# sxontheway/milliEye

Measured on AMD Instinct MI355X. Metric: frames/sec YOLOv3-416+fusion @batch32, 1/2/4/8 MI355X; mAP@0.5 vs ref, higher is better.
Workload: dtype f32; 1 GPU; yolov3.cfg 416x416 fp32 inference, batch=32 per GPU, full milliEye: Darknet.forward -> NMS -> Network.forward mode 0 (R-CNN head + radar fusion, 2 radar boxes/frame) -> output rows, synthetic frames U[0,1), deterministic trained-like weights; stage=full, batch_per_gpu=32, global_batch=32, img_size=416, parallelism=frames sharded over 1 GPU(s), one process per GPU, no data-path collective, rccl_ranks=0, full=False, output_rows_last_step=6449, rois_last_step=6449

## Files before the change

### millieye_amd/csrc/common.h

```cpp
#pragma once
#include <hip/hip_runtime.h>
#include <stdint.h>
#include <stdio.h>
#include <stdlib.h>
#include "millieye_hip.h"

namespace me {

void set_error(const char* fmt, ...);

inline int check_launch(const char* what) {
  hipError_t e = hipGetLastError();
  if (e != hipSuccess) {
    set_error("%s: %s", what, hipGetErrorString(e));
    return (int)e;
  }
  return 0;
}

inline bool aligned16(const void* p) { return (reinterpret_cast<uintptr_t>(p) & 15u) == 0; }

inline int64_t ceil_div(int64_t a, int64_t b) { return (a + b - 1) / b; }

inline int store_mode() {
  static const int mode = [] {
    const char* e = getenv("MILLIEYE_STORE_MODE");
    return e ? atoi(e) : 0;
  }();
  return mode;
}

typedef unsigned st_u32x4 __attribute__((ext_vector_type(4)));
__device__ __forceinline__ void store16(void* ptr, uint4 v, int mode) {
  if (mode == 0) {
    *reinterpret_cast<uint4*>(ptr) = v;
  } else {
    st_u32x4 d = {v.x, v.y, v.z, v.w};
    if (mode == 1)
      asm volatile("global_store_dwordx4 %0, %1, off nt" ::"v"(ptr), "v"(d) : "memory");
    else
      asm volatile("global_store_dwordx4 %0, %1, off sc1" ::"v"(ptr), "v"(d) : "memory");
  }
}
__device__ __forceinline__ void store4(float* ptr, float v, int mode) {
  if (mode == 0)
    *ptr = v;
  else
    __builtin_nontemporal_store(v, ptr);
}

}

#define ME_REQUIRE(cond, code, ...)   \
  do {                                \
    if (!(cond)) {                    \
      me::set_error(__VA_ARGS__);     \
      return (code);                  \
    }                                 \
  } while (0)

#define ME_HIP(call)                                                 \
  do {                                                               \
    hipError_t e__ = (call);                                         \
    if (e__ != hipSuccess) {                                         \
      me::set_error("%s failed: %s", #call, hipGetErrorString(e__)); \
      return (int)e__;                                               \
    }                                                                \
  } while (0)
```

### millieye_amd/csrc/conv.hip

```cpp
#include <stdlib.h>

#include "common.h"
#include "dma.h"

#include "conv32_common.h"

namespace me32 {
int launch_p8_tile(const ConvP& p, int tile, hipStream_t stream);
bool ws1x1_f32_eligible(const ConvP& p);
int launch_ws1x1_f32(const ConvP& p, hipStream_t stream);
bool ws3x3_f32_eligible(const ConvP& p);
int launch_ws3x3_f32(const ConvP& p, hipStream_t stream);
bool stem_mfma_eligible(const ConvP& p);
int launch_stem_mfma(const ConvP& p, hipStream_t stream);
}

namespace {

template <int BM, int BN, int BK, int WR, int WC, int ABL = 0, int PRIO = 0>
__global__ __launch_bounds__(256) void conv_igemm_f32(ConvP p) {
  static_assert(WR * WC == 4, "4 waves per workgroup");
  constexpr int TM = BM / WR, TN = BN / WC;
  constexpr int MT = TM / 32, NT = TN / 32;
  static_assert(MT >= 1 && NT >= 1, "wave tile must hold at least one 32x32 MFMA tile");
// ... 321 lines not shown
  const int a_row = (wr * TM + r32) * BK;
  const int b_row = (BM + wc * TN + r32) * BK;
  const int off0 = ((0 + hh) ^ sw) * 4, off1 = ((2 + hh) ^ sw) * 4;

  for (int s = 0; s < nstages; ++s) {
    if (s + 1 < nstages)
      asm volatile("s_waitcnt vmcnt(%0) lgkmcnt(0)" ::"n"(LPW) : "memory");
    else
      asm volatile("s_waitcnt vmcnt(0) lgkmcnt(0)" ::: "memory");
    __builtin_amdgcn_s_barrier();
    asm volatile("" ::: "memory");
    if (s + 2 < nstages) issue_stage((s + 2) % NST);
    if (DPRIO) __builtin_amdgcn_s_setprio(1);
    const float* Ab = smem + (s % NST) * STAGE_F + a_row;
    const float* Bb = smem + (s % NST) * STAGE_F + b_row;
    float4 af[2][MT], bf[2][NT];
#pragma unroll
    for (int half = 0; half < 2; ++half) {
      const int off = half ? off1 : off0;
#pragma unroll
      for (int i = 0; i < MT; ++i) af[half][i] = *reinterpret_cast<const float4*>(Ab + i * 32 * BK + off);
#pragma unroll
      for (int j = 0; j < NT; ++j) bf[half][j] = *reinterpret_cast<const float4*>(Bb + j * 32 * BK + off);
    }
    __builtin_amdgcn_sched_barrier(0);
#pragma unroll
    for (int half = 0; half < 2; ++half) {
#pragma unroll
      for (int kk = 0; kk < 4; ++kk)
#pragma unroll
        for (int i = 0; i < MT; ++i)
#pragma unroll
          for (int j = 0; j < NT; ++j) {
            const float4 av = af[half][i], bv = bf[half][j];
            const float a = kk == 0 ? av.x : kk == 1 ? av.y : kk == 2 ? av.z : av.w;
            const float b = kk == 0 ? bv.x : kk == 1 ? bv.y : kk == 2 ? bv.z : bv.w;
            acc[i][j] = __builtin_amdgcn_mfma_f32_32x32x2f32(a, b, acc[i][j], 0, 0, 0);
          }
    }
    if (DPRIO) __builtin_amdgcn_s_setprio(0);
  }

  if (p.splitk > 1) {
    float* slab = p.partial + (long long)sid * p.M * p.cout;
#pragma unroll
    for (int j = 0; j < NT; ++j) {
      const int co = n0 + wc * TN + j * 32 + r32;
#pragma unroll
      for (int i = 0; i < MT; ++i)
#pragma unroll
        for (int e = 0; e < 16; ++e) {
          const int m = m0 + wr * TM + i * 32 + (e & 3) + 8 * (e >> 2) + 4 * hh;
          if (co < p.cout && m < p.M) slab[(long long)m * p.cout + co] = acc[i][j][e];
        }
    }
    return;
  }
  const int hw = p.ho * p.wo;
#pragma unroll
  for (int j = 0; j < NT; ++j) {
    const int co = n0 + wc * TN + j * 32 + r32;
    const bool co_ok = co < p.cout;
    const float sc = co_ok ? p.scale[co] : 0.f;
    const float sh = co_ok ? p.shift[co] : 0.f;
#pragma unroll
    for (int i = 0; i < MT; ++i) {
#pragma unroll
      for (int e = 0; e < 16; ++e) {
        const int row = (e & 3) + 8 * (e >> 2) + 4 * hh;
        const int m = m0 + wr * TM + i * 32 + row;
        if (!co_ok || m >= p.M) continue;
        float v = apply_act(acc[i][j][e] * sc + sh, p.act);
        if (p.res) v += p.res[(long long)m * p.res_pitch + co];
        if (p.ups == 1) {
          p.y[(long long)m * p.y_pitch + co] = v;
        } else {
          const int nimg = m / hw;
          const int rem = m - nimg * hw;
          const int oy = rem / p.wo, ox = rem - oy * p.wo;
          const int W2 = p.wo * 2;
          const long long base = ((long long)nimg * (p.ho * 2) + 2 * oy) * W2 + 2 * ox;
          p.y[(base)*p.y_pitch + co] = v;
          p.y[(base + 1) * p.y_pitch + co] = v;
          p.y[(base + W2) * p.y_pitch + co] = v;
          p.y[(base + W2 + 1) * p.y_pitch + co] = v;
        }
      }
    }
  }
}

template <int CT>
__global__ __launch_bounds__(256) void conv_stem3_f32(ConvP p) {
  constexpr int K = 27;
  const int m = blockIdx.x * 256 + threadIdx.x;
  const int co0 = blockIdx.y * CT;
  if (m >= p.M) return;
  const int hw = p.ho * p.wo;
  const int nimg = m / hw;
  const int rem = m - nimg * hw;
  const int oy = rem / p.wo, ox = rem - oy * p.wo;
  float xin[K];
#pragma unroll
  for (int ky = 0; ky < 3; ++ky)
#pragma unroll
    for (int kx = 0; kx < 3; ++kx) {
      const int iy = oy * p.stride - p.pad + ky, ix = ox * p.stride - p.pad + kx;
      const bool ok = ((unsigned)iy < (unsigned)p.h) && ((unsigned)ix < (unsigned)p.w);
#pragma unroll
      for (int c = 0; c < 3; ++c) {
        float v = 0.f;
        if (ok)
          v = p.x_nchw ? p.x[(((long long)nimg * 3 + c) * p.h + iy) * p.w + ix]
                       : p.x[((long long)(nimg * p.h + iy) * p.w + ix) * p.x_pitch + c];
        xin[(ky * 3 + kx) * 3 + c] = v;
      }
    }
  const float* __restrict__ wg = p.wgt + (long long)co0 * K;
  float acc[CT];
#pragma unroll
  for (int j = 0; j < CT; ++j) {
    float a = 0.f;
#pragma unroll
    for (int k = 0; k < K; ++k) a = fmaf(xin[k], wg[j * K + k], a);
    acc[j] = apply_act(a * p.scale[co0 + j] + p.shift[co0 + j], p.act);
  }
  float* yrow = p.y + (long long)m * p.y_pitch + co0;
#pragma unroll
  for (int j = 0; j < CT; j += 4) *reinterpret_cast<float4*>(yrow + j) = make_float4(acc[j], acc[j + 1], acc[j + 2], acc[j + 3]);
}

using namespace me_dma;

__device__ __forceinline__ unsigned udiv_magic32(unsigned n, unsigned m, unsigned s) { return (__umulhi(n, m) + n) >> s; }

template <int N, class F, int I = 0>
__device__ __forceinline__ void static_for(F&& f) {
  if constexpr (I < N) {
    f(std::integral_constant<int, I>{});
    static_for<N, F, I + 1>(static_cast<F&&>(f));
  }
}

__device__ __forceinline__ void tile_coords(const ConvP& p, int t, int& tile_m, int& tile_n) {
  const int per_panel = p.tiles_m * p.gn;
  const int panel = t / per_panel;
  const int r = t - panel * per_panel;
  const int left = p.tiles_n - panel * p.gn;
  const int width = left < p.gn ? left : p.gn;
  tile_m = r / width;
  tile_n = panel * p.gn + (r - tile_m * width);
}

template <int BM, int BN, int WR, int WC, int MINW = 1, int BABL = 0, int HYB = 0, int KORD = 0, int DEEP = 0, int MASKED = 0>
__global__ __launch_bounds__(64 * WR * WC, MINW) void conv_igemm_buf_f32(ConvP p) {
  constexpr int NW = WR * WC;
  static_assert(NW == 4 || NW == 8, "4 or 8 waves per workgroup");
  constexpr int BK = 16, NST = DEEP ? (KORD ? 9 : 6) : 3;
  constexpr int DEPTH = NST - 1;
  constexpr int TM = BM / WR, TN = BN / WC;
  constexpr int MT = TM / 32, NT = TN / 32;
  constexpr int GA = BM / 16, G = (BM + BN) / 16;
  constexpr int LPW = (G + NW - 1) / NW;
  constexpr int LA = GA / NW;
  constexpr int STAGE_F = LPW * NW * 256;
  static_assert(GA % NW == 0, "A groups must split evenly over the waves");

  extern __shared__ __attribute__((aligned(16))) float smem[];
  const unsigned lds_base = (unsigned)(unsigned long long)(__attribute__((address_space(3))) float*)smem;

  const int tid = threadIdx.x;
  const int lane = tid & 63;
  const int wave = __builtin_amdgcn_readfirstlane(tid >> 6);
  const int wr = wave / WC, wc = wave % WC;
  const int r32 = lane & 31, hh = lane >> 5;

  int tile_m, tile_n;
  int sid = blockIdx.y;
  int piece = -1;
  {
    int nwg = p.tiles_m * p.tiles_n;
    int bid = blockIdx.x;
    int first = 0, per = 1;
    if constexpr (HYB) {
      if (bid < p.bulk) {
        nwg = p.bulk;
      } else {
        bid -= p.bulk;
        first = p.bulk;
        per = p.splitk;
        nwg = (nwg - p.bulk) * p.splitk;
      }
    }
    const int q = nwg >> 3, r = nwg & 7;
    const int xcd = bid & 7, idx = bid >> 3;
    int wg = (xcd < r ? xcd * (q + 1) : r * (q + 1) + (xcd - r) * q) + idx;
    if constexpr (HYB) {
      if (first || p.bulk == 0) {
        piece = wg;
        sid = wg % per;
        wg = first + wg / per;
      } else {
        sid = 0;
      }
    }
    tile_coords(p, wg, tile_m, tile_n);
    tile_m = __builtin_amdgcn_readfirstlane(tile_m);
    tile_n = __builtin_amdgcn_readfirstlane(tile_n);
  }
  const int m0 = tile_m * BM, n0 = tile_n * BN;
  const int hw = p.ho * p.wo;

  const int img0 = (int)udiv_magic32((unsigned)m0, p.hw_m, p.hw_s);
  const long long img_elems = (long long)p.h * p.w * p.x_pitch;
  const long long bias_elems = ((long long)p.pad * p.w + p.pad) * p.x_pitch;
  const u32x4 rsrc_a = make_rsrc(p.x + (long long)img0 * img_elems - bias_elems);
  const bool b_tiled = p.wgt_tiled != nullptr;
  const u32x4 rsrc_b = make_rsrc(b_tiled ? p.wgt_tiled + (long long)n0 * 16 : p.wgt + (long long)n0 * p.ktot);
  const unsigned b_row = b_tiled ? 64u : (unsigned)p.ktot * 4u;
  const unsigned b_step = b_tiled ? (unsigned)p.cout * 64u : BK * 4u;

  const int lrow = lane >> 2;
  unsigned v_base[LPW];
  constexpr bool KS3 = KORD == 1;
  unsigned v_pad[LA];
  unsigned v_cur[LPW];
#pragma unroll
  for (int j = 0; j < LPW; ++j) {
    const int g = wave + NW * j;
    const int row = g * 16 + lrow;
    const int q = (lane & 3) ^ ((row >> 2) & 3);
    v_base[j] = kOobOffset;
    if (j < LA) {
      unsigned padmask = 0xFFFFFFFFu;
      const int m = m0 + row;
      if (m < p.M) {
        const int nimg = (int)udiv_magic32((unsigned)m, p.hw_m, p.hw_s);
        const int rem = m - nimg * hw;
        const int oy = (int)udiv_magic32((unsigned)rem, p.wo_m, p.wo_s), ox = rem - oy * p.wo;
        const int iy0 = oy * p.stride - p.pad, ix0 = ox * p.stride - p.pad;
        unsigned ok = 0;
        auto in_w = [&](int kx) { return (unsigned)(ix0 + kx) < (unsigned)p.w ? 1u : 0u; };
        auto in_h = [&](int ky) { return (unsigned)(iy0 + ky) < (unsigned)p.h; };
        if (KS3 || p.ks == 3) {
          const unsigned cols = in_w(0) | in_w(1) << 1 | in_w(2) << 2;
          ok = (in_h(0) ? cols : 0u) | (in_h(1) ? cols << 3 : 0u) | (in_h(2) ? cols << 6 : 0u);
        } else if (p.ks == 1) {
          ok = in_h(0) ? in_w(0) : 0u;
        } else {
          unsigned cols = 0;
          for (int kx = 0; kx < p.ks; ++kx) cols |= in_w(kx) << kx;
          for (int ky = 0; ky < p.ks; ++ky) ok |= (in_h(ky) ? cols : 0u) << (ky * p.ks);
        }
        padmask = ~ok;
        const long long e = (long long)(nimg - img0) * img_elems + ((long long)iy0 * p.w + ix0) * p.x_pitch + bias_elems;
        v_base[j] = (unsigned)(e * 4) + 16u * q;
      }
      v_pad[j] = padmask;
    } else if (g < G) {
      const int co_local = row - BM;
      if (n0 + co_local < p.cout) v_base[j] = (unsigned)co_local * b_row + 16u * q;
    }
    v_cur[j] = BABL == 1 ? kOobOffset : v_base[j];
  }

  int s_begin = sid * p.sps;
  int s_end = (s_begin + p.sps < p.stages) ? s_begin + p.sps : p.stages;
  if constexpr (HYB) {
    if (piece < 0) {
      s_begin = 0;
      s_end = p.stages;
    }
  }
  f32x16 acc[MT][NT];
#pragma unroll
  for (int i = 0; i < MT; ++i)
#pragma unroll
    for (int j = 0; j < NT; ++j)
#pragma unroll
      for (int e = 0; e < 16; ++e) acc[i][j][e] = 0.f;

  constexpr unsigned STAGE_B = STAGE_F * 4u;
  const unsigned wave_lds = __builtin_amdgcn_readfirstlane(lds_base + (unsigned)wave * 1024u);
  const unsigned pitch4 = (unsigned)p.x_pitch * 4u;
  const int sw = (r32 >> 2) & 3;
  const int off0 = ((0 + hh) ^ sw) * 4, off1 = ((2 + hh) ^ sw) * 4;
  const float* a_frag = smem + (wr * TM + r32) * BK;
  const float* b_frag = smem + (BM + wc * TN + r32) * BK;

  auto compute_stage = [&](const float* Ab, const float* Bb) {
    if (MT * NT >= 4) __builtin_amdgcn_s_setprio(1);
    float4 af[2][MT], bf[2][NT];
#pragma unroll
    for (int half = 0; half < 2; ++half) {
      const int off = half ? off1 : off0;
#pragma unroll
      for (int i = 0; i < MT; ++i) af[half][i] = *reinterpret_cast<const float4*>(Ab + i * 32 * BK + off);
#pragma unroll
      for (int j = 0; j < NT; ++j) bf[half][j] = *reinterpret_cast<const float4*>(Bb + j * 32 * BK + off);
    }
    __builtin_amdgcn_sched_barrier(0);
#pragma unroll
    for (int half = 0; half < 2; ++half) {
#pragma unroll
      for (int kk = 0; kk < 4; ++kk)
#pragma unroll
        for (int i = 0; i < MT; ++i)
#pragma unroll
// ... 31 lines not shown
      b_off = (unsigned)tap * (unsigned)p.cs * b_step;
    };
    enter_tap();
    a_off += (unsigned)cc * (BK * 4u);
    b_off += (unsigned)cc * b_step;
    auto issue_stage = [&](unsigned lds_dst) {
      dma_stage<LPW, LA, NW * 1024>(v_cur, rsrc_a, rsrc_b, __builtin_amdgcn_readfirstlane(a_off),
                                    __builtin_amdgcn_readfirstlane(b_off), lds_dst);
      a_off += BK * 4u;
      b_off += b_step;
      if (++cc == p.cs) {
        cc = 0;
        do {
          ++tap;
          if (++kx == p.ks) {
            kx = 0;
            ++ky;
          }
        } while (MASKED && tap < p.ks * p.ks && !((tmask >> tap) & 1u));
        enter_tap();
      }
    };
    const int nstages = s_end - s_begin;
    for (int i = 0; i < DEPTH && i < nstages; ++i) issue_stage(wave_lds + (unsigned)i * STAGE_B);
    auto wait_landed = [&](int younger) {
      bool done = false;
      static_for<DEPTH>([&](auto r_c) {
        constexpr int R = decltype(r_c)::value;
        if (!done && younger <= R) {
          asm volatile("s_waitcnt vmcnt(%0) lgkmcnt(0)" ::"n"(LPW * R) : "memory");
          done = true;
        }
      });
      if (!done) asm volatile("s_waitcnt vmcnt(%0) lgkmcnt(0)" ::"n"(LPW * (DEPTH - 1)) : "memory");
    };
    auto step = [&](auto slot_c) {
      constexpr int SLOT = decltype(slot_c)::value;
      asm volatile("s_waitcnt vmcnt(%0) lgkmcnt(0)" ::"n"(LPW * (DEPTH - 1)) : "memory");
      __builtin_amdgcn_s_barrier();
      asm volatile("" ::: "memory");
      issue_stage(wave_lds + ((SLOT + DEPTH) % NST) * STAGE_B);
      compute_stage(a_frag + SLOT * STAGE_F, b_frag + SLOT * STAGE_F);
    };
    int s = 0;
    for (; s + NST <= nstages - DEPTH; s += NST) static_for<NST>(step);
    int slot = 0;
    for (; s < nstages; ++s) {
      wait_landed(nstages - 1 - s);
      __builtin_amdgcn_s_barrier();
      asm volatile("" ::: "memory");
      if (s + DEPTH < nstages) issue_stage(wave_lds + (slot == 0 ? NST - 1 : slot - 1) * STAGE_B);
      compute_stage(a_frag + slot * STAGE_F, b_frag + slot * STAGE_F);
      slot = slot == NST - 1 ? 0 : slot + 1;
    }
  } else {
    unsigned v_tap[9][LPW];
    unsigned a_tap[9], b_tap[9];
#pragma unroll
    for (int t = 0; t < 9; ++t) {
#pragma unroll
      for (int j = 0; j < LPW; ++j)
        v_tap[t][j] = j < LA ? ((BABL == 1 || ((v_pad[j < LA ? j : 0] >> t) & 1u)) ? kOobOffset : v_base[j]) : v_cur[j];
      a_tap[t] = (unsigned)((t / 3) * p.w + (t % 3)) * pitch4;
      b_tap[t] = (unsigned)t * (unsigned)p.cs * b_step;
    }
    const int c_begin = s_begin / 9, c_end = s_end / 9;
    unsigned ca = (unsigned)c_begin * (BK * 4u), cb = (unsigned)c_begin * b_step;
    auto issue = [&](auto tap_c, unsigned ca_, unsigned cb_, unsigned lds_dst) {
      constexpr int T = decltype(tap_c)::value;
      dma_stage<LPW, LA, NW * 1024>(v_tap[T], rsrc_a, rsrc_b, __builtin_amdgcn_readfirstlane(a_tap[T] + ca_),
                                    __builtin_amdgcn_readfirstlane(b_tap[T] + cb_), lds_dst);
    };
    auto step = [&](auto tap_c, auto last_c) {
      constexpr int T = decltype(tap_c)::value;
      constexpr bool LAST = decltype(last_c)::value;
      constexpr int SLOT = T % NST;
      constexpr int YOUNGER = (LAST && 8 - T < DEPTH - 1) ? 8 - T : DEPTH - 1;
      asm volatile("s_waitcnt vmcnt(%0) lgkmcnt(0)" ::"n"(LPW * YOUNGER) : "memory");
      __builtin_amdgcn_s_barrier();
      asm volatile("" ::: "memory");
      constexpr unsigned DST = ((SLOT + DEPTH) % NST) * STAGE_B;
      if constexpr (T + DEPTH < 9)
        issue(std::integral_constant<int, (T + DEPTH) % 9>{}, ca, cb, wave_lds + DST);
      else if constexpr (!LAST)
        issue(std::integral_constant<int, (T + DEPTH) % 9>{}, ca + BK * 4u, cb + b_step, wave_lds + DST);
      compute_stage(a_frag + SLOT * STAGE_F, b_frag + SLOT * STAGE_F);
    };
    auto chunk = [&](auto last_c) { static_for<9>([&](auto tap_c) { step(tap_c, last_c); }); };
    static_for<DEPTH>([&](auto tap_c) { issue(tap_c, ca, cb, wave_lds + decltype(tap_c)::value * STAGE_B); });
    for (int c = c_begin; c + 1 < c_end; ++c) {
      chunk(std::false_type{});
      ca += BK * 4u;
      cb += b_step;
    }
    chunk(std::true_type{});
  }

  const bool split = HYB ? piece >= 0 : p.splitk > 1;
  if (split) {
    const long long slab_stride = HYB ? (long long)(BM * BN) : (long long)p.M * p.cout;
    float* slab0 = HYB ? p.partial + (long long)(piece - sid) * (BM * BN) : p.partial;
    auto slab_index = [&](int i, int j, int e, long long& idx) {
      const int lm = wr * TM + i * 32 + (e & 3) + 8 * (e >> 2) + 4 * hh, lc = wc * TN + j * 32 + r32;
      if (HYB) {
        idx = (long long)lm * BN + lc;
        return true;
      }
      idx = (long long)(m0 + lm) * p.cout + (n0 + lc);
      return m0 + lm < p.M && n0 + lc < p.cout;
    };
    float* mine = slab0 + (long long)sid * slab_stride;
#pragma unroll
    for (int j = 0; j < NT; ++j)
#pragma unroll
      for (int i = 0; i < MT; ++i)
#pragma unroll
        for (int e = 0; e < 16; ++e) {
          long long idx;
          if (!slab_index(i, j, e, idx)) continue;
          if (p.counters)
            __hip_atomic_store(mine + idx, acc[i][j][e], __ATOMIC_RELAXED, __HIP_MEMORY_SCOPE_AGENT);
          else
            mine[idx] = acc[i][j][e];
        }
    if (p.counters == nullptr) return;
    asm volatile("s_waitcnt vmcnt(0)" ::: "memory");
    __syncthreads();
    int* last_flag = reinterpret_cast<int*>(smem);
    if (tid == 0) {
      int* cnt = p.counters + (HYB ? piece / p.splitk : tile_m * p.tiles_n + tile_n);
      const int ticket = __hip_atomic_fetch_add(cnt, 1, __ATOMIC_RELAXED, __HIP_MEMORY_SCOPE_AGENT);
      const int last = ticket == p.splitk - 1;
      if (last) __hip_atomic_store(cnt, 0, __ATOMIC_RELAXED, __HIP_MEMORY_SCOPE_AGENT);
      *last_flag = last;
    }
    __syncthreads();
    if (*last_flag == 0) return;
#pragma unroll
    for (int j = 0; j < NT; ++j)
#pragma unroll
      for (int i = 0; i < MT; ++i)
#pragma unroll
        for (int e = 0; e < 16; ++e) {
          long long idx;
          if (!slab_index(i, j, e, idx)) continue;
          float a = __hip_atomic_load(slab0 + idx, __ATOMIC_RELAXED, __HIP_MEMORY_SCOPE_AGENT);
          for (int k = 1; k < p.splitk; ++k)
            a += __hip_atomic_load(slab0 + (long long)k * slab_stride + idx, __ATOMIC_RELAXED, __HIP_MEMORY_SCOPE_AGENT);
          acc[i][j][e] = a;
        }
  }
  if (m0 + BM <= p.M && n0 + BN <= p.cout && p.ups == 1 && p.act != ME_ACT_SIGMOID) {
    const float slope = p.act == ME_ACT_LEAKY ? 0.1f : 1.0f;
    const long long ystep = p.y_pitch, rstep = p.res_pitch;
#pragma unroll
    for (int j = 0; j < NT; ++j) {
      const int co = n0 + wc * TN + j * 32 + r32;
      const float sc = p.scale[co], sh = p.shift[co];
#pragma unroll
      for (int i = 0; i < MT; ++i) {
        const long long row0 = m0 + wr * TM + i * 32 + 4 * hh;
        float* yp = p.y + row0 * ystep + co;
        if (p.res) {
          const float* rp = p.res + row0 * rstep + co;
#pragma unroll
          for (int e = 0; e < 16; ++e) {
            const float t = acc[i][j][e] * sc + sh;
            me::store4(yp, fmaxf(t, t * slope) + *rp, p.store_mode);
            yp += (e & 3) == 3 ? 5 * ystep : ystep;
            rp += (e & 3) == 3 ? 5 * rstep : rstep;
          }
        } else {
#pragma unroll
          for (int e = 0; e < 16; ++e) {
            const float t = acc[i][j][e] * sc + sh;
            me::store4(yp, fmaxf(t, t * slope), p.store_mode);
            yp += (e & 3) == 3 ? 5 * ystep : ystep;
          }
        }
      }
    }
    return;
  }
#pragma unroll
  for (int j = 0; j < NT; ++j) {
    const int co = n0 + wc * TN + j * 32 + r32;
    const bool co_ok = co < p.cout;
    const float sc = co_ok ? p.scale[co] : 0.f;
    const float sh = co_ok ? p.shift[co] : 0.f;
#pragma unroll
    for (int i = 0; i < MT; ++i) {
#pragma unroll
      for (int e = 0; e < 16; ++e) {
        const int row = (e & 3) + 8 * (e >> 2) + 4 * hh;
        const int m = m0 + wr * TM + i * 32 + row;
        if (!co_ok || m >= p.M) continue;
        float v = apply_act(acc[i][j][e] * sc + sh, p.act);
        if (p.res) v += p.res[(long long)m * p.res_pitch + co];
        if (p.ups == 1) {
          p.y[(long long)m * p.y_pitch + co] = v;
        } else {
          const int nimg = m / hw;
          const int rem = m - nimg * hw;
          const int oy = rem / p.wo, ox = rem - oy * p.wo;
          const int W2 = p.wo * 2;
          const long long base = ((long long)nimg * (p.ho * 2) + 2 * oy) * W2 + 2 * ox;
          p.y[(base)*p.y_pitch + co] = v;
          p.y[(base + 1) * p.y_pitch + co] = v;
          p.y[(base + W2) * p.y_pitch + co] = v;
          p.y[(base + W2 + 1) * p.y_pitch + co] = v;
        }
      }
    }
  }
}

__global__ __launch_bounds__(256) void conv_splitk_reduce_f32(ConvP p) {
  const long long total = (long long)p.M * p.cout;
  const int hw = p.ho * p.wo;
  for (long long idx = (long long)blockIdx.x * 256 + threadIdx.x; idx < total; idx += (long long)gridDim.x * 256) {
    const int co = (int)(idx % p.cout);
    const int m = (int)(idx / p.cout);
    float a = p.partial[idx];
    for (int k = 1; k < p.splitk; ++k) a += p.partial[(long long)k * total + idx];
    float v = apply_act(a * p.scale[co] + p.shift[co], p.act);
    if (p.res) v += p.res[(long long)m * p.res_pitch + co];
    if (p.ups == 1) {
      p.y[(long long)m * p.y_pitch + co] = v;
    } else {
      const int nimg = m / hw;
      const int rem = m - nimg * hw;
      const int oy = rem / p.wo, ox = rem - oy * p.wo;
      const int W2 = p.wo * 2;
      const long long base = ((long long)nimg * (p.ho * 2) + 2 * oy) * W2 + 2 * ox;
      p.y[(base)*p.y_pitch + co] = v;
      p.y[(base + 1) * p.y_pitch + co] = v;
      p.y[(base + W2) * p.y_pitch + co] = v;
      p.y[(base + W2 + 1) * p.y_pitch + co] = v;
    }
  }
}

__global__ __launch_bounds__(256) void conv_tail_reduce_f32(ConvP p, int bm, int bn) {
  const int tile_elems = bm * bn;
  const long long total = (long long)(p.tiles_m * p.tiles_n - p.bulk) * tile_elems;
  const int hw = p.ho * p.wo;
  for (long long idx = (long long)blockIdx.x * 256 + threadIdx.x; idx < total; idx += (long long)gridDim.x * 256) {
    const int t = (int)(idx / tile_elems);
    const int rem_e = (int)(idx - (long long)t * tile_elems);
    const int lm = rem_e / bn, lc = rem_e - lm * bn;
    int tile_m, tile_n;
    tile_coords(p, p.bulk + t, tile_m, tile_n);
    const int m = tile_m * bm + lm;
    const int co = tile_n * bn + lc;
    if (m >= p.M || co >= p.cout) continue;
    const float* src = p.partial + (long long)t * p.splitk * tile_elems + rem_e;
    float a = src[0];
    for (int k = 1; k < p.splitk; ++k) a += src[(long long)k * tile_elems];
    float v = apply_act(a * p.scale[co] + p.shift[co], p.act);
    if (p.res) v += p.res[(long long)m * p.res_pitch + co];
    if (p.ups == 1) {
      p.y[(long long)m * p.y_pitch + co] = v;
    } else {
      const int nimg = m / hw;
      const int rem = m - nimg * hw;
      const int oy = rem / p.wo, ox = rem - oy * p.wo;
      const int W2 = p.wo * 2;
      const long long base = ((long long)nimg * (p.ho * 2) + 2 * oy) * W2 + 2 * ox;
      p.y[(base)*p.y_pitch + co] = v;
      p.y[(base + 1) * p.y_pitch + co] = v;
      p.y[(base + W2) * p.y_pitch + co] = v;
      p.y[(base + W2 + 1) * p.y_pitch + co] = v;
    }
  }
}

constexpr int SC_MAXCOUT = 128;

template <int CIN>
__global__ __launch_bounds__(256) void conv_smallcin_f32(ConvP p) {
  constexpr int K = 9 * CIN;
  __shared__ __attribute__((aligned(16))) float w_lds[K * SC_MAXCOUT];
  const int cout_pad = (p.cout + 7) & ~7;
  for (int idx = threadIdx.x; idx < K * cout_pad; idx += 256) {
    const int k = idx / cout_pad, co = idx - k * cout_pad;
    const int t = k / CIN, c = k - t * CIN;
    w_lds[idx] = (co < p.cout && c < p.cin) ? p.wgt[(long long)co * (9 * p.cin) + t * p.cin + c] : 0.f;
  }
  __syncthreads();

  const int tpp = cout_pad >> 3;
  const long long gid = (long long)blockIdx.x * 256 + threadIdx.x;
  const int m = (int)(gid / tpp);
  const int co0 = (int)(gid - (long long)m * tpp) * 8;
  if (m >= p.M) return;
  const int hw = p.ho * p.wo;
  const int nimg = m / hw;
  const int rem = m - nimg * hw;
  const int oy = rem / p.wo, ox = rem - oy * p.wo;

  float xin[K];
#pragma unroll
  for (int ky = 0; ky < 3; ++ky)
#pragma unroll
    for (int kx = 0; kx < 3; ++kx) {
      const int iy = oy * p.stride - p.pad + ky, ix = ox * p.stride - p.pad + kx;
// ... 205 lines not shown
  return a_max < (1ll << 31) && b_max < (1ll << 31) && b_tiled_max < (1ll << 31) && (long long)p.x_pitch * 4 < (1ll << 31);
}

void magic_u32(unsigned d, unsigned* m, unsigned* s) {
  unsigned sh = 0;
  while ((1ull << sh) < d) ++sh;
  *s = sh;
  *m = (unsigned)(((1ull << 32) * ((1ull << sh) - d)) / d + 1);
}

template <int BN>
void choose_order(ConvP& p) {
  static const long long kPanelBytes = [] {
    const char* e = getenv("MILLIEYE_PANEL_KB");
    return (e && atoi(e) > 0 ? (long long)atoi(e) : 1300ll) * 1024;
  }();
  static const int kChunkMajor = [] {
    const char* e = getenv("MILLIEYE_KORD");
    return e ? atoi(e) : 2;
  }();
  const long long col_bytes = (long long)BN * p.ktot * 4;
  p.gn = p.tiles_n;
  p.kord = (p.ks == 3 && p.cs >= 4 && kChunkMajor == 2) ? 1 : 0;
  if (col_bytes * p.tiles_n > kPanelBytes) {
    const long long fit = kPanelBytes / col_bytes;
    p.gn = fit < 1 ? 1 : fit > p.tiles_n ? p.tiles_n : (int)fit;
    if (p.ks == 3 && kChunkMajor >= 1) p.kord = 1;
  }
}

template <int BM, int BN, int WR, int WC, int MINW, int BABL, int HYB, int KORD, int DEEP = 0, int MASKED = 0>
int launch_buf_kernel(const ConvP& p, dim3 grid, hipStream_t stream) {
  constexpr int NW = WR * WC;
  constexpr int LPW = ((BM + BN) / 16 + NW - 1) / NW;
  constexpr int NST = DEEP ? (KORD ? 9 : 6) : 3;
  const size_t lds = (size_t)NST * LPW * NW * 256 * sizeof(float);
  auto kern = conv_igemm_buf_f32<BM, BN, WR, WC, MINW, BABL, HYB, KORD, DEEP, MASKED>;
  if (lds > 64 * 1024) {
    static bool attr_set = false;
    if (!attr_set) {
      ME_HIP(hipFuncSetAttribute(reinterpret_cast<const void*>(kern), hipFuncAttributeMaxDynamicSharedMemorySize,
                                 (int)lds));
      attr_set = true;
    }
  }
  hipLaunchKernelGGL(kern, grid, dim3(64 * NW), lds, stream, p);
  return me::check_launch(HYB ? "conv_igemm_buf_f32<tail split>" : "conv_igemm_buf_f32");
}

template <int BM, int BN, int WR, int WC, int MINW = 1, int BABL = 0, int DEEP = 0>
int launch_buf(ConvP& p, hipStream_t stream) {
  if (p.ks * p.ks > 32) {
    if constexpr (WR * WC == 4)
      return launch_igemm<BM, BN, 16, WR, WC>(p, stream);
    else
      return launch_igemm<128, 128, 16, 2, 2>(p, stream);
  }
  if (p.mask_cols)
    ME_REQUIRE(buf_addressable<BM>(p) && p.mask_cols % BN == 0 && BABL == 0 && DEEP == 0, ME_E_BADARG,
               "me_conv2d_f32: tap masks need cin %% 16 == 0, offsets below 2^31 and a tile width (%d) that divides tap_mask_cols", BN);
  if (!buf_addressable<BM>(p)) return launch_dma<BM, BN, WR, WC, 1, MINW>(p, stream);
  constexpr int BK = 16;
  p.cs = (p.cin + BK - 1) / BK;
  p.stages = p.ks * p.ks * p.cs;
  p.tiles_m = (p.M + BM - 1) / BM;
  p.tiles_n = (p.cout + BN - 1) / BN;
  choose_order<BN>(p);
  if (BABL || p.mask_cols) p.kord = 0;
  plan_split(p);
  const long long blocks = (long long)p.tiles_m * p.tiles_n;
  ME_REQUIRE(blocks < (1ll << 31), ME_E_TOOBIG, "me_conv2d_f32: grid too large");
  const dim3 grid((unsigned)blocks, (unsigned)p.splitk);
  if (blocks > p.counters_len || p.splitk == 1) p.counters = nullptr;
  int rc;
  if constexpr (BABL == 0) {
    if (p.mask_cols) {
      if constexpr (DEEP == 0) rc = launch_buf_kernel<BM, BN, WR, WC, MINW, 0, 0, 0, 0, 1>(p, grid, stream);
      else rc = ME_E_BADARG;
    } else
      rc = p.kord ? launch_buf_kernel<BM, BN, WR, WC, MINW, 0, 0, 1, DEEP>(p, grid, stream)
                  : launch_buf_kernel<BM, BN, WR, WC, MINW, 0, 0, 0, DEEP>(p, grid, stream);
  } else {
    rc = launch_buf_kernel<BM, BN, WR, WC, MINW, BABL, 0, 0>(p, grid, stream);
  }
  if (rc || p.splitk == 1 || p.counters) return rc;
  long long rb = ((long long)p.M * p.cout + 255) / 256;
  if (rb > 256 * 16) rb = 256 * 16;
  hipLaunchKernelGGL(conv_splitk_reduce_f32, dim3((unsigned)rb), dim3(256), 0, stream, p);
  return me::check_launch("conv_splitk_reduce_f32");
}

template <int BM, int BN, int WR, int WC, int MINW = 1, int DEEP = 0>
int launch_buf_tail(ConvP& p, hipStream_t stream, long long ws_bytes) {
  ME_REQUIRE(p.ks * p.ks <= 32 && buf_addressable<BM>(p), ME_E_BADARG,
             "me_conv2d_f32: the tail-split tiles need cin %% 16 == 0 and offsets below 2^31");
  constexpr int BK = 16;
  p.cs = (p.cin + BK - 1) / BK;
  p.stages = p.ks * p.ks * p.cs;
  p.tiles_m = (p.M + BM - 1) / BM;
  p.tiles_n = (p.cout + BN - 1) / BN;
  choose_order<BN>(p);
  const long long tiles = (long long)p.tiles_m * p.tiles_n;
  ME_REQUIRE(tiles < (1ll << 24), ME_E_TOOBIG, "me_conv2d_f32: grid too large");
  plan_split(p);
  p.bulk = (int)(tiles / 256 * 256);
  const long long tail = tiles - p.bulk;
  if (tail == 0 || p.splitk <= 1) {
    p.splitk = 1;
    p.bulk = 0;
    return launch_buf<BM, BN, WR, WC, MINW, 0, DEEP>(p, stream);
  }
  const long long need = tail * p.splitk * BM * BN * (long long)sizeof(float);
  ME_REQUIRE(p.partial && ws_bytes >= need, ME_E_BADARG, "me_conv2d_f32: tail split %d needs a workspace of %lld bytes",
             p.splitk, need);
  const dim3 grid((unsigned)(p.bulk + tail * p.splitk));
  if (tail > p.counters_len) p.counters = nullptr;
  int rc = p.kord ? launch_buf_kernel<BM, BN, WR, WC, MINW, 0, 1, 1, DEEP>(p, grid, stream)
                  : launch_buf_kernel<BM, BN, WR, WC, MINW, 0, 1, 0, DEEP>(p, grid, stream);
  if (rc || p.counters) return rc;
  long long rb = (tail * BM * BN + 255) / 256;
  if (rb > 256 * 16) rb = 256 * 16;
  hipLaunchKernelGGL(conv_tail_reduce_f32, dim3((unsigned)rb), dim3(256), 0, stream, p, BM, BN);
  return me::check_launch("conv_tail_reduce_f32");
}

int fill_params(const me_conv_desc* d, ConvP& p) {
  p.store_mode = me::store_mode();
  ME_REQUIRE(d != nullptr, ME_E_NULLPTR, "me_conv2d_f32: null descriptor");
  ME_REQUIRE(d->n > 0 && d->h > 0 && d->w > 0 && d->cin > 0 && d->cout > 0, ME_E_BADARG,
             "me_conv2d_f32: non-positive dimension");
  ME_REQUIRE(d->ksize >= 1 && d->stride >= 1 && d->pad >= 0, ME_E_BADARG, "me_conv2d_f32: bad ksize/stride/pad");
  const int ho = (d->h + 2 * d->pad - d->ksize) / d->stride + 1;
  const int wo = (d->w + 2 * d->pad - d->ksize) / d->stride + 1;
  ME_REQUIRE(ho == d->ho && wo == d->wo, ME_E_BADARG, "me_conv2d_f32: ho/wo (%d,%d) != derived (%d,%d)", d->ho,
             d->wo, ho, wo);
  ME_REQUIRE((long long)d->n * d->ho * d->wo < (1ll << 31), ME_E_TOOBIG, "me_conv2d_f32: too many output pixels");
  p.x = d->x; p.wgt = d->wgt; p.wgt_tiled = d->wgt_tiled; p.scale = d->scale; p.shift = d->shift; p.res = d->res; p.y = d->y;
  p.x_pitch = d->x_pitch; p.res_pitch = d->res_pitch; p.y_pitch = d->y_pitch;
  p.n = d->n; p.h = d->h; p.w = d->w; p.cin = d->cin; p.cout = d->cout; p.ks = d->ksize;
  p.stride = d->stride; p.pad = d->pad; p.ho = d->ho; p.wo = d->wo; p.act = d->act; p.ups = d->upsample;
  p.x_nchw = d->x_nchw;
  p.M = d->n * d->ho * d->wo;
  p.ktot = d->ksize * d->ksize * d->cin;
  magic_u32((unsigned)(d->ho * d->wo), &p.hw_m, &p.hw_s);
  magic_u32((unsigned)d->wo, &p.wo_m, &p.wo_s);
  p.cs = p.stages = p.tiles_m = p.tiles_n = p.bulk = p.gn = p.kord = 0;
  p.partial = nullptr;
  p.splitk = 1;
  p.sps = 0;
  p.counters = d->tile_counters_len > 0 ? d->tile_counters : nullptr;
  p.counters_len = p.counters ? d->tile_counters_len : 0;
  p.mask_cols = d->tap_mask_cols > 0 ? d->tap_mask_cols : 0;
  for (int i = 0; i < 4; ++i) p.tapmask[i] = d->tap_mask[i];
  return 0;
}

}

extern "C" {

int64_t me_conv2d_flops(const me_conv_desc* d) {
  if (!d) return 0;
  return 2ll * d->n * d->ho * d->wo * (int64_t)d->cout * d->ksize * d->ksize * d->cin;
}

int64_t me_conv2d_workspace_bytes(const me_conv_desc* d) {
  ConvP p;
  if (!d || fill_params(d, p) != 0 || d->cin <= 4) return 0;
  if ((d->tile >= 41 && d->tile <= 45) || d->tile == 47) {
    static const int shape[7][2] = {{128, 128}, {128, 64}, {64, 64}, {128, 32}, {256, 128}, {0, 0}, {64, 64}};
    const int bm = shape[d->tile - 41][0], bn = shape[d->tile - 41][1];
    const long long tiles = (long long)((p.M + bm - 1) / bm) * ((p.cout + bn - 1) / bn);
    const int split = d->split_k > 0 ? d->split_k : 4;
    return (int64_t)(tiles % 256) * split * bm * bn * (int64_t)sizeof(float);
  }
  const ConvPlan plan = plan_conv(p, d->tile, d->split_k > 0 ? d->split_k : kMaxSplit);
  const int split = d->split_k > 0 ? d->split_k : plan.splitk;
  return split > 1 ? (int64_t)split * p.M * p.cout * (int64_t)sizeof(float) : 0;
}

int me_conv2d_f32(const me_conv_desc* d, void* stream_) {
  hipStream_t stream = reinterpret_cast<hipStream_t>(stream_);
  ConvP p;
  int rc = fill_params(d, p);
  if (rc) return rc;
  ME_REQUIRE(d->x && d->wgt && d->scale && d->shift && d->y, ME_E_NULLPTR, "me_conv2d_f32: null tensor pointer");
  ME_REQUIRE(d->upsample == 1 || d->upsample == 2, ME_E_BADARG, "me_conv2d_f32: upsample must be 1 or 2");
  ME_REQUIRE(d->act >= 0 && d->act <= 2, ME_E_BADARG, "me_conv2d_f32: unknown activation %d", d->act);
  ME_REQUIRE(d->y_pitch >= d->cout, ME_E_BADARG, "me_conv2d_f32: y_pitch < cout");

  if (d->cin <= 4) {
    ME_REQUIRE(d->ksize == 3, ME_E_BADARG, "me_conv2d_f32: cin <= 4 needs ksize 3 (direct stem kernel)");
    ME_REQUIRE(d->cout <= SC_MAXCOUT, ME_E_TOOBIG, "me_conv2d_f32: small-cin kernel supports cout <= %d", SC_MAXCOUT);
    ME_REQUIRE(d->res == nullptr && d->upsample == 1, ME_E_BADARG,
               "me_conv2d_f32: small-cin kernel has no residual/upsample epilogue");
    ME_REQUIRE(d->x_nchw || d->x_pitch >= d->cin, ME_E_BADARG, "me_conv2d_f32: x_pitch < cin");
    ME_REQUIRE(me::aligned16(d->y), ME_E_ALIGN, "me_conv2d_f32: y not 16-byte aligned");
    if (d->tile == 0 && me32::stem_mfma_eligible(p)) return me32::launch_stem_mfma(p, stream);
    if (d->cin == 3 && (d->y_pitch & 3) == 0 && d->tile != 91) {
      const unsigned mb = (unsigned)((p.M + 255) / 256);
      if (d->cout % 32 == 0) {
        hipLaunchKernelGGL(conv_stem3_f32<32>, dim3(mb, d->cout / 32), dim3(256), 0, stream, p);
        return me::check_launch("conv_stem3_f32");
      }
      if (d->cout % 16 == 0) {
        hipLaunchKernelGGL(conv_stem3_f32<16>, dim3(mb, d->cout / 16), dim3(256), 0, stream, p);
        return me::check_launch("conv_stem3_f32");
      }
    }
    const long long threads = (long long)p.M * (((p.cout + 7) & ~7) >> 3);
    const unsigned blocks = (unsigned)((threads + 255) / 256);
    if (d->cin == 3)
      hipLaunchKernelGGL(conv_smallcin_f32<3>, dim3(blocks), dim3(256), 0, stream, p);
    else
      hipLaunchKernelGGL(conv_smallcin_f32<4>, dim3(blocks), dim3(256), 0, stream, p);
    return me::check_launch("conv_smallcin_f32");
  }

  ME_REQUIRE(!d->x_nchw, ME_E_BADARG, "me_conv2d_f32: NCHW input only supported for cin <= 4");
  ME_REQUIRE(d->cin % 4 == 0, ME_E_BADARG, "me_conv2d_f32: cin %% 4 != 0 (cin=%d)", d->cin);
  ME_REQUIRE(d->x_pitch >= d->cin && d->x_pitch % 4 == 0, ME_E_ALIGN, "me_conv2d_f32: x_pitch must be >= cin, %% 4");
  ME_REQUIRE(me::aligned16(d->x) && me::aligned16(d->wgt), ME_E_ALIGN, "me_conv2d_f32: x / wgt not 16-byte aligned");
  ME_REQUIRE(!d->res || d->res_pitch >= d->cout, ME_E_BADARG, "me_conv2d_f32: res_pitch < cout");
  ME_REQUIRE(d->split_k >= 0 && d->split_k <= 64, ME_E_BADARG, "me_conv2d_f32: split_k out of range");

  if (p.mask_cols) {
    const int taps = d->ksize * d->ksize, classes = d->cout / p.mask_cols;
    ME_REQUIRE(taps <= 16 && d->cout % p.mask_cols == 0 && classes >= 1 && classes <= 4 && d->upsample == 1 && d->split_k <= 1 &&
                   d->tile >= 0 && d->tile <= 5 && d->cin % 16 == 0, ME_E_BADARG,
               "me_conv2d_f32: tap masks need ksize^2 <= 16, 1 - 4 column classes, upsample 1, split_k <= 1, tile 0 - 5, cin %% 16 == 0");
    for (int i = 0; i < classes; ++i)
      ME_REQUIRE((d->tap_mask[i] & ((1u << taps) - 1u)) != 0, ME_E_BADARG, "me_conv2d_f32: tap_mask[%d] selects no tap", i);
    p.splitk = 1;
    p.partial = nullptr;
    int tile = d->tile;
    if (tile == 0) tile = p.mask_cols % 128 == 0 ? 1 : p.mask_cols % 64 == 0 ? 2 : 4;
    switch (tile) {
      case 1: return launch_buf<128, 128, 2, 2>(p, stream);
      case 2: return launch_buf<128, 64, 2, 2>(p, stream);
      case 3: return launch_buf<64, 64, 2, 2>(p, stream);
      case 4: return launch_buf<128, 32, 4, 1>(p, stream);
      default: return launch_buf<256, 128, 4, 2, 4>(p, stream);
    }
  }

  if ((d->tile >= 41 && d->tile <= 45) || d->tile == 47) {
    p.splitk = d->split_k > 0 ? d->split_k : 4;
    p.partial = reinterpret_cast<float*>(d->workspace);
    const long long ws = d->workspace ? d->workspace_bytes : 0;
    switch (d->tile) {
      case 41: return launch_buf_tail<128, 128, 2, 2>(p, stream, ws);
      case 42: return launch_buf_tail<128, 64, 2, 2>(p, stream, ws);
      case 43: return launch_buf_tail<64, 64, 2, 2>(p, stream, ws);
      case 44: return launch_buf_tail<128, 32, 4, 1>(p, stream, ws);
      case 47: return launch_buf_tail<64, 64, 2, 2, 1, 1>(p, stream, ws);
      default: return launch_buf_tail<256, 128, 4, 2, 4>(p, stream, ws);
    }
  }

  const long long slab = (long long)p.M * p.cout * (long long)sizeof(float);
  int max_split = 1;
  if (d->workspace && d->workspace_bytes >= 2 * slab) {
    const long long fit = d->workspace_bytes / slab;
    max_split = fit < kMaxSplit ? (int)fit : kMaxSplit;
  }
  ConvPlan plan = plan_conv(p, d->tile, max_split);
  if (d->split_k > 0) {
    ME_REQUIRE(d->split_k == 1 || (d->workspace && d->workspace_bytes >= d->split_k * slab), ME_E_BADARG,
               "me_conv2d_f32: split_k=%d needs a workspace of %lld bytes", d->split_k, d->split_k * slab);
    plan.splitk = d->split_k;
  }
  p.splitk = plan.splitk;
  p.partial = reinterpret_cast<float*>(d->workspace);
  if (plan.tile >= 100) return me32::launch_p8_tile(p, plan.tile, stream);
  if (plan.tile == 50 || plan.tile == 60) {
    ME_REQUIRE(d->split_k <= 1, ME_E_BADARG, "me_conv2d_f32: tile %d has no split-K form", plan.tile);
    return plan.tile == 50 ? me32::launch_ws1x1_f32(p, stream) : me32::launch_ws3x3_f32(p, stream);
  }
  switch (plan.tile) {
    case 1: return launch_buf<128, 128, 2, 2>(p, stream);
    case 2: return launch_buf<128, 64, 2, 2>(p, stream);
    case 3: return launch_buf<64, 64, 2, 2>(p, stream);
    case 4: return launch_buf<128, 32, 4, 1>(p, stream);
    case 5: return launch_buf<256, 128, 4, 2, 4>(p, stream);
    case 7: return launch_buf<64, 64, 2, 2, 1, 0, 1>(p, stream);
    case 21: return launch_dma<128, 128, 2, 2, 1>(p, stream);
    case 22: return launch_dma<128, 64, 2, 2, 1>(p, stream);
    case 23: return launch_dma<64, 64, 2, 2, 1>(p, stream);
    case 24: return launch_dma<128, 32, 4, 1, 1>(p, stream);
    case 25: return launch_dma<256, 128, 4, 2, 1, 4>(p, stream);
    case 6: return launch_dma<256, 128, 4, 2, 1, 1>(p, stream);
    case 81: return launch_buf<128, 128, 2, 2, 1, 1>(p, stream);
    case 82: return launch_buf<128, 64, 2, 2, 1, 1>(p, stream);
    case 83: return launch_buf<64, 64, 2, 2, 1, 1>(p, stream);
    case 85: return launch_buf<256, 128, 4, 2, 4, 1>(p, stream);
    case 61: return launch_dma<128, 128, 2, 2, 1, 1, 1>(p, stream);
    case 65: return launch_dma<256, 128, 4, 2, 1, 4, 1>(p, stream);
    case 51: return launch_igemm<128, 128, 16, 2, 2>(p, stream);
    case 52: return launch_igemm<128, 64, 16, 2, 2>(p, stream);
    case 53: return launch_igemm<64, 64, 16, 2, 2>(p, stream);
    case 54: return launch_igemm<128, 32, 16, 4, 1>(p, stream);
    case 55: return launch_igemm<128, 128, 32, 2, 2>(p, stream);
    case 31: return launch_igemm<128, 128, 16, 2, 2, 0, 1>(p, stream);
    case 11: return launch_igemm<128, 128, 16, 2, 2, 1>(p, stream);
    case 12: return launch_igemm<128, 128, 16, 2, 2, 2>(p, stream);
    case 13: return launch_igemm<128, 128, 16, 2, 2, 3>(p, stream);
// ... 7 lines not shown
```

### millieye_amd/csrc/conv32_common.h

```cpp
#pragma once
#include <math.h>
#include "common.h"
#include "dma.h"

typedef float f32x16 __attribute__((ext_vector_type(16)));

struct ConvP {
  const float* x;
  const float* wgt;
  const float* wgt_tiled;
  const float* scale;
  const float* shift;
  const float* res;
  float* y;
  long long x_pitch, res_pitch, y_pitch;
  int n, h, w, cin, cout, ks, stride, pad, ho, wo, act, ups, x_nchw;
  unsigned hw_m, hw_s, wo_m, wo_s;
  int M;
  int ktot;
  int cs;
  int stages;
  int tiles_m, tiles_n;
  float* partial;
  int splitk;
  int sps;
  int gn;
  int kord;
  int* counters;
  long long counters_len;
  int bulk;
  int store_mode;
  unsigned tapmask[4];
  int mask_cols;
};

__device__ __forceinline__ float apply_act(float v, int act) {
  if (act == ME_ACT_LEAKY) return v > 0.f ? v : 0.1f * v;
  if (act == ME_ACT_SIGMOID) return 1.f / (1.f + expf(-v));
  return v;
}
```

Before: 1882 frames/s.

## Stage conv epilogue through LDS for 16-byte vectorized stores and set occupancy bounds

Adds an LDS-transposed epilogue to the buffered conv kernel. Each wave writes its MFMA accumulator tile to shared memory and reads it back in row-contiguous float4 chunks, so BN/leaky/residual is applied per float4 and written with 16-byte global stores instead of scalar strided stores. It is enabled by default when pointers and pitches are aligned. It also derives per-shape minimum waves in launch_bounds, which caps register use to raise occupancy at some risk of spills. The change adds a barrier, LDS traffic and s_nop after the inline-asm stores.

```diff
diff --git a/millieye_amd/csrc/common.h b/millieye_amd/csrc/common.h
--- a/millieye_amd/csrc/common.h
+++ b/millieye_amd/csrc/common.h
@@ -30,6 +30,14 @@
   return mode;
 }
 
+inline int epilogue16() {
+  static const int on = [] {
+    const char* e = getenv("MILLIEYE_EPILOGUE16");
+    return e ? atoi(e) != 0 : 1;
+  }();
+  return on;
+}
+
 typedef unsigned st_u32x4 __attribute__((ext_vector_type(4)));
 __device__ __forceinline__ void store16(void* ptr, uint4 v, int mode) {
   if (mode == 0) {
@@ -37,9 +45,9 @@
   } else {
     st_u32x4 d = {v.x, v.y, v.z, v.w};
     if (mode == 1)
-      asm volatile("global_store_dwordx4 %0, %1, off nt" ::"v"(ptr), "v"(d) : "memory");
+      asm volatile("global_store_dwordx4 %0, %1, off nt\n\ts_nop 1" ::"v"(ptr), "v"(d) : "memory");
     else
-      asm volatile("global_store_dwordx4 %0, %1, off sc1" ::"v"(ptr), "v"(d) : "memory");
+      asm volatile("global_store_dwordx4 %0, %1, off sc1\n\ts_nop 1" ::"v"(ptr), "v"(d) : "memory");
   }
 }
 __device__ __forceinline__ void store4(float* ptr, float v, int mode) {
diff --git a/millieye_amd/csrc/conv.hip b/millieye_amd/csrc/conv.hip
--- a/millieye_amd/csrc/conv.hip
+++ b/millieye_amd/csrc/conv.hip
@@ -497,8 +497,13 @@
   tile_n = panel * p.gn + (r - tile_m * width);
 }
 
+constexpr int buf_min_waves(int bm, int bn, int wr, int wc, int minw, bool hyb_or_masked) {
+  const int per_wave = (bm / wr) * (bn / wc);
+  return minw != 1 ? minw : per_wave == 1024 ? 6 : per_wave == 2048 && hyb_or_masked ? 4 : 1;
+}
+
 template <int BM, int BN, int WR, int WC, int MINW = 1, int BABL = 0, int HYB = 0, int KORD = 0, int DEEP = 0, int MASKED = 0>
-__global__ __launch_bounds__(64 * WR * WC, MINW) void conv_igemm_buf_f32(ConvP p) {
+__global__ __launch_bounds__(64 * WR * WC, buf_min_waves(BM, BN, WR, WC, MINW, HYB || MASKED)) void conv_igemm_buf_f32(ConvP p) {
   constexpr int NW = WR * WC;
   static_assert(NW == 4 || NW == 8, "4 or 8 waves per workgroup");
   constexpr int BK = 16, NST = DEEP ? (KORD ? 9 : 6) : 3;
@@ -836,6 +841,82 @@
   }
   if (m0 + BM <= p.M && n0 + BN <= p.cout && p.ups == 1 && p.act != ME_ACT_SIGMOID) {
     const float slope = p.act == ME_ACT_LEAKY ? 0.1f : 1.0f;
+    if (p.ep16) {
+      __syncthreads();
+      float* img = smem + wave * 1024;
+      float* wp = img + hh * 128 + r32;
+      const float4* rp4 = reinterpret_cast<const float4*>(img) + lane;
+      const int lrow8 = lane >> 3, lcol = 4 * (lane & 7);
+      const unsigned yoff = ((unsigned)lrow8 * (unsigned)p.y_pitch + (unsigned)lcol) * 4u;
+      const unsigned roff = ((unsigned)lrow8 * (unsigned)p.res_pitch + (unsigned)lcol) * 4u;
+      const long long roww = m0 + wr * TM;
+      const int colw = n0 + wc * TN;
+      char* ybase = reinterpret_cast<char*>(p.y + roww * p.y_pitch + colw);
+      const char* rbase = reinterpret_cast<const char*>(p.res + roww * p.res_pitch + colw);
+      const unsigned ypitch4 = (unsigned)p.y_pitch * 4u, rpitch4 = (unsigned)p.res_pitch * 4u;
+      auto tile = [&](auto res_c, auto plain_c) {
+        constexpr bool RES = decltype(res_c)::value, PLAIN = decltype(plain_c)::value;
+#pragma unroll
+        for (int j = 0; j < NT; ++j) {
+          const float4 sc = *reinterpret_cast<const float4*>(p.scale + colw + j * 32 + lcol);
+          const float4 sh = *reinterpret_cast<const float4*>(p.shift + colw + j * 32 + lcol);
+#pragma unroll
+          for (int i = 0; i < MT; ++i) {
+#pragma unroll
+            for (int e = 0; e < 16; ++e) wp[((e & 3) + 8 * (e >> 2)) * 32] = acc[i][j][e];
+            asm volatile("s_waitcnt lgkmcnt(0)" ::: "memory");
+            float4 rr[4];
+            if constexpr (RES) {
+#pragma unroll
+              for (int k = 0; k < 4; ++k) {
+                const unsigned row = (unsigned)(i * 32 + 8 * k) * rpitch4 + j * 128;
+                rr[k] = *reinterpret_cast<const float4*>(rbase + (roff + row));
+              }
+            }
+            __builtin_amdgcn_sched_barrier(0);
+            float4 v[4];
+#pragma unroll
+            for (int k = 0; k < 4; ++k) v[k] = rp4[64 * k];
+            asm volatile("" ::: "memory");
+            __builtin_amdgcn_sched_barrier(0);
+            auto one = [&](float a, float s, float h) {
+              const float t = a * s + h;
+              return fmaxf(t, t * slope);
+            };
+#pragma unroll
+            for (int k = 0; k < 4; ++k) {
+              float4 o;
+              o.x = one(v[k].x, sc.x, sh.x);
+              o.y = one(v[k].y, sc.y, sh.y);
+              o.z = one(v[k].z, sc.z, sh.z);
+              o.w = one(v[k].w, sc.w, sh.w);
+              if constexpr (RES) {
+                o.x += rr[k].x;
+                o.y += rr[k].y;
+                o.z += rr[k].z;
+                o.w += rr[k].w;
+              }
+              const unsigned row = (unsigned)(i * 32 + 8 * k) * ypitch4 + j * 128;
+              me::store16(ybase + (yoff + row), make_uint4(__float_as_uint(o.x), __float_as_uint(o.y), __float_as_uint(o.z), __float_as_uint(o.w)),
+                          PLAIN ? 0 : p.store_mode);
+              __builtin_amdgcn_sched_barrier(0);
+            }
+          }
+        }
+      };
+      if (p.store_mode == 0) {
+        if (p.res)
+          tile(std::true_type{}, std::true_type{});
+        else
+          tile(std::false_type{}, std::true_type{});
+      } else {
+        if (p.res)
+          tile(std::true_type{}, std::false_type{});
+        else
+          tile(std::false_type{}, std::false_type{});
+      }
+      return;
+    }
     const long long ystep = p.y_pitch, rstep = p.res_pitch;
 #pragma unroll
     for (int j = 0; j < NT; ++j) {
@@ -1347,6 +1428,9 @@
   p.counters_len = p.counters ? d->tile_counters_len : 0;
   p.mask_cols = d->tap_mask_cols > 0 ? d->tap_mask_cols : 0;
   for (int i = 0; i < 4; ++i) p.tapmask[i] = d->tap_mask[i];
+  auto rows16 = [](const float* ptr, long long pitch) { return me::aligned16(ptr) && pitch % 4 == 0 && pitch < (1ll << 22); };
+  p.ep16 = me::epilogue16() && d->upsample == 1 && d->act != ME_ACT_SIGMOID && rows16(d->y, d->y_pitch) &&
+           (!d->res || rows16(d->res, d->res_pitch)) && me::aligned16(d->scale) && me::aligned16(d->shift);
   return 0;
 }
 
diff --git a/millieye_amd/csrc/conv32_common.h b/millieye_amd/csrc/conv32_common.h
--- a/millieye_amd/csrc/conv32_common.h
+++ b/millieye_amd/csrc/conv32_common.h
@@ -32,6 +32,7 @@
   int store_mode;
   unsigned tapmask[4];
   int mask_cols;
+  int ep16;
 };
 
 __device__ __forceinline__ float apply_act(float v, int act) {
```

Result: faster. 1927 frames/s (median of 6 runs) (+2.4%).
